# pyxploiter/HandMvNet

Measured on AMD Instinct MI355X. Metric: samples/sec (BxV frames) eval_fps.py, 8-view 256x256; 21-kpt L2 vs reference, higher is better.
Workload: dtype f32; 1 GPU; BASELINE configs[2]: B=32/GPU x V=8 x 256x256, resnet50_paper backbone, d=524, cross_attn x5, GCN decoder; global_batch=32, views=8, frame=256, parallelism=sample-shard x1

## Files before the change

handmvnet_amd/csrc/conv_stream.hip:

```cpp
#include <cstdio>
#include <cstdlib>
#include <type_traits>
#include <utility>

#include "kernels.h"

namespace hmv {

typedef float sf32x16 __attribute__((ext_vector_type(16)));
typedef float sf32x4 __attribute__((ext_vector_type(4)));
typedef _Float16 sf16x8 __attribute__((ext_vector_type(8)));

#define HMV_SGLDS16(gptr, lptr)                                                                             \
    __builtin_amdgcn_global_load_lds((const __attribute__((address_space(1))) void *)(gptr),                \
                                     (__attribute__((address_space(3))) void *)(lptr), 16, 0, 0)

template <int N>
__device__ __forceinline__ void wait_vm() {
    static_assert(N >= 0 && N < 64, "vmcnt is a 6-bit field");
    asm volatile("s_waitcnt vmcnt(%0)" ::"n"(N) : "memory");
}
template <typename F, int... I>
__device__ __forceinline__ void static_for_impl(F &&f, std::integer_sequence<int, I...>) {
    (f(std::integral_constant<int, I>{}), ...);
}
template <int N, typename F>
__device__ __forceinline__ void static_for(F &&f) {
    static_for_impl(static_cast<F &&>(f), std::make_integer_sequence<int, N>{});
}

constexpr int sched_r(int RB, int RS, int j) { return RS ? RS : (j == 0 ? RB : 0); }
constexpr int sched_ops(int NP, int PA, int RB, int RS, int OS, int slot) { return slot < NP ? PA + sched_r(RB, RS, slot) : OS; }
constexpr int sched_after_piece(int NP, int D, int PA, int RB, int RS, int OS, int j) {
    const int T0 = 8, g = T0 * NP + j - D, tq = g / NP, jq = g - tq * NP;
    int n = sched_r(RB, RS, jq);
    for (int s = tq * (NP + 1) + jq + 1; s < T0 * (NP + 1) + j; ++s) n += sched_ops(NP, PA, RB, RS, OS, s % (NP + 1));
    return n;
}
constexpr int sched_after_residual(int NP, int PA, int RB, int RS, int OS) {
    const int T0 = 8, last = RS ? NP - 1 : 0;
    int n = 0;
    for (int s = (T0 - 1) * (NP + 1) + last + 1; s < T0 * (NP + 1) + NP; ++s) n += sched_ops(NP, PA, RB, RS, OS, s % (NP + 1));
    return n;
}
static_assert(sched_after_piece(4, 3, 1, 8, 0, 8, 0) == 10 && sched_after_piece(4, 3, 1, 8, 0, 8, 1) == 18 && sched_after_piece(4, 3, 1, 8, 0, 8, 2) == 18 &&
              sched_after_piece(4, 3, 1, 8, 0, 8, 3) == 10 && sched_after_residual(4, 1, 8, 0, 8) == 23, "the step-0 schedule of four pieces, counted by hand");
static_assert(sched_after_piece(4, 3, 1, 8, 2, 8, 0) == 2 + 3 + 3 + 8 && sched_after_residual(4, 1, 8, 2, 8) == 8 + 4 * 3, "the spread K = 256 schedule");

template <int TM, int TN, int MW, int NW, int NP, int NSLOT, bool HAS_RES, bool SPREAD = false, bool DUAL = false, int N2 = 0>
__global__ __launch_bounds__(64 * MW *NW, (MW * NW) / 4) void conv_stream_f16(const ConvParams p) {
    constexpr int NWV = MW * NW, NT = 64 * NWV;
    constexpr int BM = 32 * TM * MW, BN = 32 * TN * NW;
    constexpr int D = NSLOT - 1;
    constexpr int PA = BM * 8 / NT;
    constexpr int NB2 = N2 / 32;
    constexpr int TM2 = N2 ? (BM / 32) * NB2 / NWV : 0;
    constexpr int K2Q = BN / 16;
    static_assert(N2 == 0 || (N2 % 32 == 0 && TN == 2 && TM2 >= 1 && NWV % NB2 == 0 && (BM / 32) == (NWV / NB2) * TM2),
                  "chain: a wave's 64 output channels are one pixel piece of the second reduction; whole blocks per wave");
    constexpr int RB = HAS_RES ? TM * TN * 2 : 0, OS = TM * TN * 2 + 2 * TM2;
    constexpr int RS = (SPREAD && HAS_RES) ? RB / NP : 0;
    static_assert(!SPREAD || RB % NP == 0, "spread schedule: whole residual DMAs per step");
    constexpr int ZW = TM * TN * 2 * 1024;
    constexpr int NFAKE = (D + NP - 1) / NP;
    static_assert(NT == 512 && BM % 64 == 0 && PA >= 1, "eight waves; whole DMA passes per piece");
    static_assert((NSLOT & (NSLOT - 1)) == 0 && NSLOT >= 2, "a power of two");
    extern __shared__ __attribute__((aligned(16))) char ssm[];
    _Float16 *sA = reinterpret_cast<_Float16 *>(ssm);
    char *zones = ssm + NSLOT * BM * 128;

    const int tid = threadIdx.x, lane = tid & 63;
    const int wave = __builtin_amdgcn_readfirstlane(tid >> 6);
    const int l31 = lane & 31, kh = lane >> 5;
    const int mw = wave / NW, nw = wave - mw * NW;
    const int zi = N2 ? nw * MW + mw : wave;
    static_assert(N2 == 0 || !HAS_RES || ZW == TM * 32 * 128, "chain: a landing zone is the wave's region of the tile image");

    const int nsl = p.ntiles;
    const int loc = (int)blockIdx.x >> 3, per_xcd = 32 / nsl;
    const int slice = loc % nsl, stream = ((int)blockIdx.x & 7) * per_xcd + loc / nsl, nstreams = 8 * per_xcd;
    const int ntl = p.mtiles > stream ? (p.mtiles - stream + nstreams - 1) / nstreams : 0;
    if (ntl == 0) return;
    const int n0 = slice * BN + nw * TN * 32;

    const _Float16 *zero16 = reinterpret_cast<const _Float16 *>(p.zero);
    _Float16 *trash = reinterpret_cast<_Float16 *>(const_cast<float *>(p.zero) + 64 + 4 * lane);
    const _Float16 *Ain = reinterpret_cast<const _Float16 *>(p.in);
    const _Float16 *Rin = reinterpret_cast<const _Float16 *>(p.res);
    _Float16 *Out = reinterpret_cast<_Float16 *>(p.out);

    const int wl31 = (l31 & 0x13) | ((l31 & 4) << 1) | ((l31 & 8) >> 1);
    sf16x8 wreg[TN][NP * 4];
    {
        const _Float16 *wb = reinterpret_cast<const _Float16 *>(p.wgt) + (size_t)(n0 + wl31) * p.ldw + 8 * kh;
#pragma unroll
        for (int b = 0; b < TN; ++b)
#pragma unroll
            for (int Q = 0; Q < NP * 4; ++Q) wreg[b][Q] = *reinterpret_cast<const sf16x8 *>(wb + (size_t)(32 * b) * p.ldw + 16 * Q);
    }
    const int ob2 = N2 ? wave % (N2 ? NB2 : 1) : 0, pg2 = N2 ? wave / (N2 ? NB2 : 1) : 0;
    sf16x8 w2reg[N2 ? K2Q : 1];
    if constexpr (N2 > 0) {
        const _Float16 *wb2 = reinterpret_cast<const _Float16 *>(p.nx_wgt) + (size_t)(32 * ob2 + wl31) * p.nx_ldw + 8 * kh;
#pragma unroll
        for (int Q = 0; Q < K2Q; ++Q) w2reg[Q] = *reinterpret_cast<const sf16x8 *>(wb2 + 16 * Q);
    }
    asm volatile("s_waitcnt vmcnt(0)" ::: "memory");

    const int arow = tid >> 3, kqs = (tid & 7) ^ ((tid >> 4) & 7);
    const int fsw = (l31 >> 1) & 7;

    size_t off2[DUAL ? PA : 1] = {};
    auto issue_A = [&](int G) {
        const int tt = G >= 0 ? G / NP : -1, jj = G >= 0 ? G - tt * NP : 0, slot = G & (NSLOT - 1);
        const int mt = stream + tt * nstreams;
#pragma unroll
        for (int i = 0; i < PA; ++i) {
            const int m = mt * BM + i * 64 + arow;
            const bool ok = tt >= 0 && tt < ntl && m < p.M;
            const _Float16 *src = zero16;
            if constexpr (DUAL) {
                if (jj * 64 == p.ksplit) {
                    const int hw = p.Ho * p.Wo, n = m / hw, rem = m - n * hw, ho = rem / p.Wo, wo = rem - ho * p.Wo;
                    off2[i] = ((size_t)(n * p.H2 + ho * p.stride2) * p.W2 + wo * p.stride2) * p.lda2 + 8 * kqs;
                }
                if (ok && jj * 64 >= p.ksplit) {
                    src = reinterpret_cast<const _Float16 *>(p.in2) + off2[i] + (jj * 64 - p.ksplit);
                } else if (ok) {
                    src = Ain + (size_t)m * p.lda + jj * 64 + 8 * kqs;
                }
            } else if (ok) {
                src = Ain + (size_t)m * p.lda + jj * 64 + 8 * kqs;
            }
            asm volatile("" : "+v"(src));
            HMV_SGLDS16(src, sA + ((slot * BM + i * 64 + wave * 8) * 64));
        }
    };
    auto issue_R = [&](int tt, auto first_c, auto count_c) {
        if constexpr (HAS_RES) {
            constexpr int first = decltype(first_c)::value, count = decltype(count_c)::value;
            const int mt = stream + tt * nstreams;
            char *z = zones + ((tt & 1) * NWV + zi) * ZW;
#pragma unroll
            for (int idx = first; idx < first + count; ++idx) {
                const int a = idx / (2 * TN), b = (idx / 2) % TN, j = idx & 1;
                const int m = mt * BM + (mw * TM + a) * 32 + l31;
                const bool ok = tt >= 0 && tt < ntl && m < p.M;
                const _Float16 *src = ok ? Rin + (size_t)m * p.ldr + n0 + 32 * b + 16 * j + 8 * kh : zero16;
                asm volatile("" : "+v"(src));
                HMV_SGLDS16(src, z + idx * 1024);
            }
        }
    };
    using I0 = std::integral_constant<int, 0>;
    using IRB = std::integral_constant<int, RB>;
    using IRS = std::integral_constant<int, RS>;

#pragma unroll
    for (int ft = -NFAKE; ft < 0; ++ft) {
        static_for<NP>([&](auto jc) {
            constexpr int j = decltype(jc)::value;
            issue_A(ft * NP + j + D);
            if constexpr (RS > 0) issue_R(ft + 1, std::integral_constant<int, j * RS>{}, IRS{});
            else if constexpr (j == 0) issue_R(ft + 1, I0{}, IRB{});
        });
#pragma unroll
        for (int i = 0; i < OS; ++i)
            asm volatile("global_store_dwordx4 %0, %1, off\n\ts_nop 1" ::"v"(trash), "v"(sf32x4{0.f, 0.f, 0.f, 0.f}) : "memory");
    }

    const float lo = (p.act == ACT_RELU) ? 0.f : -INFINITY;
    const __attribute__((address_space(4))) float *bp0 =
        (const __attribute__((address_space(4))) float *)(p.bias + __builtin_amdgcn_readfirstlane(n0));
    sf32x16 acc[TM][TN];

    for (int tt = 0; tt < ntl; ++tt) {
        int bz;
        asm volatile("s_mov_b32 %0, 0" : "=s"(bz));
        const __attribute__((address_space(4))) float *bp = bp0 + bz;
#pragma unroll
        for (int b = 0; b < TN; ++b)
#pragma unroll
            for (int e = 0; e < 16; ++e) {
                const int c = 32 * b + 16 * (e >> 3) + (e & 7);
                const float v0 = bp[c], v1 = bp[c + 8];
                const float v = kh ? v1 : v0;
#pragma unroll
                for (int a = 0; a < TM; ++a) acc[a][b][e] = v;
            }
        static_for<NP>([&](auto jc) {
            constexpr int j = decltype(jc)::value;
            wait_vm<sched_after_piece(NP, D, PA, RB, RS, OS, j)>();
            asm volatile("s_waitcnt lgkmcnt(0)\n\ts_barrier" ::: "memory");
            issue_A(tt * NP + j + D);
            if constexpr (RS > 0) issue_R(tt + 1, std::integral_constant<int, j * RS>{}, IRS{});
            else if constexpr (j == 0) issue_R(tt + 1, I0{}, IRB{});
            const _Float16 *pa = sA + ((((tt * NP + j) & (NSLOT - 1)) * BM + mw * TM * 32 + l31) * 64);
#pragma unroll
            for (int q = 0; q < 4; ++q) {
                sf16x8 px[TM];
#pragma unroll
                for (int a = 0; a < TM; ++a) px[a] = *reinterpret_cast<const sf16x8 *>(pa + a * 32 * 64 + (((2 * q + kh) ^ fsw) * 8));
#pragma unroll
                for (int a = 0; a < TM; ++a)
#pragma unroll
                    for (int b = 0; b < TN; ++b)
                        acc[a][b] = __builtin_amdgcn_mfma_f32_32x32x16_f16(wreg[b][4 * j + q], px[a], acc[a][b], 0, 0, 0);
            }
        });
        if constexpr (HAS_RES) wait_vm<sched_after_residual(NP, PA, RB, RS, OS)>();
        const int mt = stream + tt * nstreams;
        const char *z = zones + ((tt & 1) * NWV + zi) * ZW + lane * 16;
        if constexpr (N2 > 0) {
            char *yt = HAS_RES ? zones + (tt & 1) * NWV * ZW : zones;
            sf16x8 rr[TM][TN][2], hv[TM][TN][2];
            if constexpr (HAS_RES) {
#pragma unroll
                for (int a = 0; a < TM; ++a)
#pragma unroll
                    for (int b = 0; b < TN; ++b)
#pragma unroll
                        for (int j = 0; j < 2; ++j) rr[a][b][j] = *reinterpret_cast<const sf16x8 *>(z + ((a * TN + b) * 2 + j) * 1024);
            }
#pragma unroll
            for (int a = 0; a < TM; ++a) {
                const int m = mt * BM + (mw * TM + a) * 32 + l31;
                _Float16 *orow = Out + (size_t)m * p.ldc + n0 + 8 * kh;
#pragma unroll
                for (int b = 0; b < TN; ++b)
#pragma unroll
                    for (int j = 0; j < 2; ++j) {
                        sf16x8 r = {0, 0, 0, 0, 0, 0, 0, 0};
                        if constexpr (HAS_RES) r = rr[a][b][j];
#pragma unroll
                        for (int u = 0; u < 8; ++u) hv[a][b][j][u] = (_Float16)fmaxf(acc[a][b][8 * j + u] * p.acc_scale + (float)r[u], lo);
                        _Float16 *dst = m < p.M ? orow + 32 * b + 16 * j : trash;
                        asm volatile("global_store_dwordx4 %0, %1, off\n\ts_nop 1" ::"v"(dst), "v"(hv[a][b][j]) : "memory");
                        if constexpr (!HAS_RES) {
                            const unsigned ya = (unsigned)(size_t)(__attribute__((address_space(3))) char *)yt +
                                                (unsigned)((nw * BM + (mw * TM + a) * 32 + l31) * 128 + (((4 * b + 2 * j + kh) ^ fsw) * 16));
                            asm volatile("ds_write_b128 %0, %1" ::"v"(ya), "v"(hv[a][b][j]) : "memory");
                        }
                    }
            }
            if constexpr (HAS_RES) {
#pragma unroll
            for (int a = 0; a < TM; ++a)
#pragma unroll
                for (int b = 0; b < TN; ++b)
#pragma unroll
                    for (int j = 0; j < 2; ++j) {
                        const unsigned ya = (unsigned)(size_t)(__attribute__((address_space(3))) char *)yt +
                                            (unsigned)((nw * BM + (mw * TM + a) * 32 + l31) * 128 + (((4 * b + 2 * j + kh) ^ fsw) * 16));
                        asm volatile("ds_write_b128 %0, %1" ::"v"(ya), "v"(hv[a][b][j]) : "memory");
                    }
            }
            asm volatile("s_waitcnt lgkmcnt(0)\n\ts_barrier" ::: "memory");
            const __attribute__((address_space(4))) float *bq =
                (const __attribute__((address_space(4))) float *)(p.nx_bias + __builtin_amdgcn_readfirstlane(32 * ob2)) + bz;
            sf32x16 acc2[TM2];
#pragma unroll
            for (int e = 0; e < 16; ++e) {
                const int c = 16 * (e >> 3) + (e & 7);
                const float v0 = bq[c], v1 = bq[c + 8];
                const float v = kh ? v1 : v0;
#pragma unroll
                for (int a = 0; a < TM2; ++a) acc2[a][e] = v;
            }
            const unsigned yr = (unsigned)(size_t)(__attribute__((address_space(3))) char *)yt + (unsigned)((pg2 * TM2 * 32 + l31) * 128);
            constexpr int G = 4 / TM2, NG = K2Q / G;
            static_assert(K2Q % G == 0 && G * TM2 == 4, "four fragment reads per group");
            sf16x8 px[2][G][TM2];
#define HMV_CHAIN_READ_GROUP(g)                                                                                                     \
    _Pragma("unroll") for (int i = 0; i < G; ++i) _Pragma("unroll") for (int a = 0; a < TM2; ++a) {                                \
        const int Q = (g) * G + i;                                                                                                  \
        const unsigned ad = yr + (unsigned)(((Q >> 2) * BM + a * 32) * 128) + (unsigned)((((2 * (Q & 3) + kh) ^ fsw)) * 16);        \
        asm volatile("ds_read_b128 %0, %1" : "=v"(px[(g) & 1][i][a]) : "v"(ad) : "memory");                                         \
    }
            HMV_CHAIN_READ_GROUP(0)
#pragma unroll
            for (int g = 0; g < NG; ++g) {
                sf16x8(&pg)[G][TM2] = px[g & 1];
                if (g + 1 < NG) {
                    HMV_CHAIN_READ_GROUP(g + 1)
                    if constexpr (TM2 == 1) asm volatile("s_waitcnt lgkmcnt(4)" : "+v"(pg[0][0]), "+v"(pg[1][0]), "+v"(pg[2][0]), "+v"(pg[3][0]) :: "memory");
                    else asm volatile("s_waitcnt lgkmcnt(4)" : "+v"(pg[0][0]), "+v"(pg[0][1]), "+v"(pg[1][0]), "+v"(pg[1][1]) :: "memory");
                } else {
                    if constexpr (TM2 == 1) asm volatile("s_waitcnt lgkmcnt(0)" : "+v"(pg[0][0]), "+v"(pg[1][0]), "+v"(pg[2][0]), "+v"(pg[3][0]) :: "memory");
                    else asm volatile("s_waitcnt lgkmcnt(0)" : "+v"(pg[0][0]), "+v"(pg[0][1]), "+v"(pg[1][0]), "+v"(pg[1][1]) :: "memory");
                }
#pragma unroll
                for (int i = 0; i < G; ++i)
#pragma unroll
                    for (int a = 0; a < TM2; ++a) acc2[a] = __builtin_amdgcn_mfma_f32_32x32x16_f16(w2reg[g * G + i], pg[i][a], acc2[a], 0, 0, 0);
            }
#undef HMV_CHAIN_READ_GROUP
            const float lo2 = (p.nx_act == ACT_RELU) ? 0.f : -INFINITY;
            _Float16 *Out2 = reinterpret_cast<_Float16 *>(p.nx_out);
#pragma unroll
            for (int a = 0; a < TM2; ++a) {
                const int m = mt * BM + (pg2 * TM2 + a) * 32 + l31;
                _Float16 *orow = Out2 + (size_t)m * p.nx_ldc + 32 * ob2 + 8 * kh;
#pragma unroll
                for (int j = 0; j < 2; ++j) {
                    const sf16x8 r = {0, 0, 0, 0, 0, 0, 0, 0};
                    sf16x8 h2;
#pragma unroll
                    for (int u = 0; u < 8; ++u) h2[u] = (_Float16)fmaxf(acc2[a][8 * j + u] * p.acc_scale + (float)r[u], lo2);
                    _Float16 *dst = m < p.M ? orow + 16 * j : trash;
                    asm volatile("global_store_dwordx4 %0, %1, off\n\ts_nop 1" ::"v"(dst), "v"(h2) : "memory");
                }
            }
        } else {
#pragma unroll
        for (int a = 0; a < TM; ++a) {
            const int m = mt * BM + (mw * TM + a) * 32 + l31;
            _Float16 *orow = Out + (size_t)m * p.ldc + n0 + 8 * kh;
#pragma unroll
            for (int b = 0; b < TN; ++b)
#pragma unroll
                for (int j = 0; j < 2; ++j) {
                    sf16x8 r = {0, 0, 0, 0, 0, 0, 0, 0};
                    if constexpr (HAS_RES) r = *reinterpret_cast<const sf16x8 *>(z + ((a * TN + b) * 2 + j) * 1024);
                    sf16x8 hv;
#pragma unroll
                    for (int u = 0; u < 8; ++u) hv[u] = (_Float16)fmaxf(acc[a][b][8 * j + u] * p.acc_scale + (float)r[u], lo);
                    _Float16 *dst = m < p.M ? orow + 32 * b + 16 * j : trash;
                    asm volatile("global_store_dwordx4 %0, %1, off\n\ts_nop 1" ::"v"(dst), "v"(hv) : "memory");
                }
        }
        }
    }
    asm volatile("s_waitcnt vmcnt(0) lgkmcnt(0)" ::: "memory");
}

template <int TM, int TN, int MW, int NW, int NP, int NSLOT, bool HAS_RES, bool DUAL = false, bool HALF = false>
__global__ __launch_bounds__(64 * MW *NW, 2) void conv_stream_f32(const ConvParams p) {
    constexpr int NWV = MW * NW, NT = 64 * NWV;
    constexpr int BM = 32 * TM * MW, BN = 32 * TN * NW;
    constexpr int D = NSLOT - 1;
    constexpr int PA = BM * 8 / NT;
    constexpr int RB = HAS_RES ? TM * TN * 4 : 0, OS = TM * TN * 4, RS = 0;
    constexpr int ZW = TM * TN * 4 * 1024;
    constexpr int NFAKE = (D + NP - 1) / NP;
    constexpr int RPP = NT / 8;
    static_assert((NT == 512 || (HALF && NT == 256)) && BM % RPP == 0 && PA >= 1 && (!HALF || (HAS_RES && !DUAL)), "whole DMA passes per piece");
    static_assert((NSLOT & (NSLOT - 1)) == 0 && NSLOT >= 2, "a power of two");
    extern __shared__ __attribute__((aligned(16))) char ssm[];
    float *sA = reinterpret_cast<float *>(ssm);
    char *zones = ssm + NSLOT * BM * 128;

    const int tid = threadIdx.x, lane = tid & 63;
    const int wave = __builtin_amdgcn_readfirstlane(tid >> 6);
    const int l31 = lane & 31, kh = lane >> 5;
    const int mw = wave / NW, nw = wave - mw * NW;
    const int nsl = p.ntiles;
    const int loc = (int)blockIdx.x >> 3, per_xcd = ((int)gridDim.x >> 3) / nsl;
    const int slice = loc % nsl, stream = ((int)blockIdx.x & 7) * per_xcd + loc / nsl, nstreams = 8 * per_xcd;
    const int ntl = p.mtiles > stream ? (p.mtiles - stream + nstreams - 1) / nstreams : 0;
    if (ntl == 0) return;
    const int n0 = slice * BN + nw * TN * 32;

    const float *zero32 = p.zero;
    float *trash = const_cast<float *>(p.zero) + 64 + 4 * lane;
    const float *Ain = reinterpret_cast<const float *>(p.in);
    const float *Rin = reinterpret_cast<const float *>(p.res);
    float *Out = reinterpret_cast<float *>(p.out);

    sf32x4 wreg[TN][NP * 4], bias[TN][4];
    {
        const float *wb = reinterpret_cast<const float *>(p.wgt) + (size_t)(n0 + l31) * p.ldw + 4 * kh;
#pragma unroll
        for (int b = 0; b < TN; ++b) {
#pragma unroll
            for (int Q = 0; Q < NP * 4; ++Q) wreg[b][Q] = *reinterpret_cast<const sf32x4 *>(wb + (size_t)(32 * b) * p.ldw + 8 * Q);
#pragma unroll
            for (int g = 0; g < 4; ++g) bias[b][g] = *reinterpret_cast<const sf32x4 *>(p.bias + n0 + 32 * b + 8 * g + 4 * kh);
        }
    }
    asm volatile("s_waitcnt vmcnt(0)" ::: "memory");

    const int arow = tid >> 3, kqs = (tid & 7) ^ ((tid >> 4) & 7);
    const int fsw = (l31 >> 1) & 7;
    auto issue_A = [&](int G) {
        const int tt = G >= 0 ? G / NP : -1, jj = G >= 0 ? G - tt * NP : 0, slot = G & (NSLOT - 1);
        const int mt = stream + tt * nstreams;
#pragma unroll
        for (int i = 0; i < PA; ++i) {
            const int m = mt * BM + i * RPP + arow;
            const bool ok = tt >= 0 && tt < ntl && m < p.M;
            const float *src = zero32;
            if constexpr (DUAL) {
                if (ok && jj * 32 >= p.ksplit) {
                    const int hw = p.Ho * p.Wo, n = m / hw, rem = m - n * hw, ho = rem / p.Wo, wo = rem - ho * p.Wo;
                    src = reinterpret_cast<const float *>(p.in2) + ((size_t)(n * p.H2 + ho * p.stride2) * p.W2 + wo * p.stride2) * p.lda2 +
                          (jj * 32 - p.ksplit) + 4 * kqs;
                } else if (ok) {
                    src = Ain + (size_t)m * p.lda + jj * 32 + 4 * kqs;
                }
            } else if (ok) {
                src = Ain + (size_t)m * p.lda + jj * 32 + 4 * kqs;
            }
            asm volatile("" : "+v"(src));
            HMV_SGLDS16(src, sA + ((slot * BM + i * RPP + wave * 8) * 32));
        }
    };
    auto issue_R = [&](int tt) {
        if constexpr (HAS_RES) {
            const int mt = stream + tt * nstreams;
            char *z = zones + ((HALF ? 0 : (tt & 1)) * NWV + wave) * ZW;
#pragma unroll
            for (int idx = 0; idx < RB; ++idx) {
                const int a = idx / (4 * TN), b = (idx / 4) % TN, g = idx & 3;
                const int m = mt * BM + (mw * TM + a) * 32 + l31;
                const bool ok = tt >= 0 && tt < ntl && m < p.M;
                const float *src = ok ? Rin + (size_t)m * p.ldr + n0 + 32 * b + 8 * g + 4 * kh : zero32;
                asm volatile("" : "+v"(src));
                HMV_SGLDS16(src, z + idx * 1024);
            }
        }
    };
#pragma unroll
    for (int ft = -NFAKE; ft < 0; ++ft) {
        static_for<NP>([&](auto jc) {
            constexpr int j = decltype(jc)::value;
            issue_A(ft * NP + j + D);
            if constexpr (j == 0) issue_R(HALF ? ft : ft + 1);
        });
#pragma unroll
        for (int i = 0; i < OS; ++i)
            asm volatile("global_store_dwordx4 %0, %1, off\n\ts_nop 1" ::"v"(trash), "v"(sf32x4{0.f, 0.f, 0.f, 0.f}) : "memory");
    }

    const float lo = (p.act == ACT_RELU) ? 0.f : -INFINITY;
    sf32x16 acc[TM][TN];
    for (int tt = 0; tt < ntl; ++tt) {
#pragma unroll
        for (int a = 0; a < TM; ++a)
#pragma unroll
            for (int b = 0; b < TN; ++b)
#pragma unroll
                for (int e = 0; e < 16; ++e) acc[a][b][e] = 0.f;
        static_for<NP>([&](auto jc) {
            constexpr int j = decltype(jc)::value;
            wait_vm<sched_after_piece(NP, D, PA, RB, RS, OS, j)>();
            asm volatile("s_waitcnt lgkmcnt(0)\n\ts_barrier" ::: "memory");
            issue_A(tt * NP + j + D);
            if constexpr (j == 0) issue_R(HALF ? tt : tt + 1);
            const float *pa = sA + ((((tt * NP + j) & (NSLOT - 1)) * BM + mw * TM * 32 + l31) * 32);
#pragma unroll
            for (int q = 0; q < 4; ++q) {
                sf32x4 px[TM];
#pragma unroll
                for (int a = 0; a < TM; ++a) px[a] = *reinterpret_cast<const sf32x4 *>(pa + a * 32 * 32 + (((2 * q + kh) ^ fsw) * 4));
#pragma unroll
                for (int e = 0; e < 4; ++e)
#pragma unroll
                    for (int a = 0; a < TM; ++a)
#pragma unroll
                        for (int b = 0; b < TN; ++b)
                            acc[a][b] = __builtin_amdgcn_mfma_f32_32x32x2f32(wreg[b][4 * j + q][e], px[a][e], acc[a][b], 0, 0, 0);
            }
        });
        if constexpr (HAS_RES) wait_vm<HALF ? (NP - 1) * PA : sched_after_residual(NP, PA, RB, RS, OS)>();
        const int mt = stream + tt * nstreams;
        const char *z = zones + ((HALF ? 0 : (tt & 1)) * NWV + wave) * ZW + lane * 16;
#pragma unroll
        for (int a = 0; a < TM; ++a) {
            const int m = mt * BM + (mw * TM + a) * 32 + l31;
            float *orow = Out + (size_t)m * p.ldc + n0 + 4 * kh;
#pragma unroll
            for (int b = 0; b < TN; ++b)
#pragma unroll
                for (int g = 0; g < 4; ++g) {
                    sf32x4 r = {0.f, 0.f, 0.f, 0.f};
                    if constexpr (HAS_RES) r = *reinterpret_cast<const sf32x4 *>(z + ((a * TN + b) * 4 + g) * 1024);
                    sf32x4 t;
#pragma unroll
                    for (int u = 0; u < 4; ++u) t[u] = fmaxf((acc[a][b][4 * g + u] + bias[b][g][u]) + r[u], lo);
                    float *dst = m < p.M ? orow + 32 * b + 8 * g : trash;
                    asm volatile("global_store_dwordx4 %0, %1, off\n\ts_nop 1" ::"v"(dst), "v"(t) : "memory");
                }
        }
    }
    asm volatile("s_waitcnt vmcnt(0) lgkmcnt(0)" ::: "memory");
}

template <int TM, int TN, int MW, int NW, int NP, int NSLOT, bool HAS_RES, bool SPREAD = false, bool DUAL = false, int N2 = 0>
static hipError_t launch_stream_one(ConvParams p, hipStream_t s) {
    constexpr int BM = 32 * TM * MW, BN = 32 * TN * NW, NWV = MW * NW;
    constexpr size_t lds = (size_t)NSLOT * BM * 128 + (HAS_RES ? (size_t)2 * NWV * TM * TN * 2 * 1024 : (N2 ? (size_t)BM * BN * 2 : 0));
    static_assert(lds <= 160 * 1024, "LDS budget");
    auto kern = conv_stream_f16<TM, TN, MW, NW, NP, NSLOT, HAS_RES, SPREAD, DUAL, N2>;
    if (N2 && (p.Cout != BN || p.nx_cout != N2 || !p.nx_wgt || !p.nx_bias || !p.nx_out)) return hipErrorInvalidValue;
    static DeviceOnce once;
    if (const hipError_t e = once.run([&](int) { return set_max_lds(lds, kern); }); e != hipSuccess) return e;
    p.mtiles = (p.M + BM - 1) / BM;
    p.ntiles = p.Cout / BN;
    hipLaunchKernelGGL(kern, dim3(256), dim3(64 * NWV), lds, s, p);
    return hipGetLastError();
}

static int stream_bn(const ConvParams &p, int *bm = nullptr) {
    int bn = 0, m = 0;
    if (p.in2) {
        if (!p.res && p.Kpad == 128 && p.ksplit == 64 && p.Cout == 256) { bn = 256; m = 128; }
        else if (!p.res && p.Kpad == 384 && p.ksplit == 128 && p.Cout == 512) { bn = 256; m = 64; }
    } else if (p.res) {
        if (p.Kpad == 256 || p.Kpad == 128) { bn = 512; m = 64; }
        else if (p.Kpad == 64) { bn = 256; m = 128; }
    } else {
        if (p.Kpad == 256 && p.Cout == 64) { bn = 64; m = 256; }
        else if (p.Kpad == 512 && p.Cout == 128) { bn = 128; m = 128; }
        else if (p.Kpad == 256 && p.Cout == 128) { bn = 128; m = 128; }
        else if (p.Kpad == 64 && p.Cout == 64) { bn = 64; m = 256; }
    }
    if (bm) *bm = m;
    return bn;
}

static int stream32_shape(const ConvParams &p) {
    if (p.in_f16 || p.out_f16) return 0;
    if (p.in2) return (!p.res && p.Kpad == 128 && p.ksplit == 64 && p.Cout == 256 && p.lda == p.ksplit && p.lda2 % 4 == 0) ? 3 : 0;
    if (p.res) return (!p.res_f16 && (p.Kpad == 64 || p.Kpad == 128 || p.Kpad == 256) && p.Cout % 256 == 0 && 32 % (p.Cout / 256) == 0) ? 1 : 0;
    return (p.Kpad == 256 && p.Cout == 64) ? 2 : ((p.Kpad == 64 && p.Cout == 64) ? 4 : 0);
}
static bool stream32_rule(const ConvParams &p) {
    static const bool no256 = HMV_DEV_ENV("HMV_NO_STREAM32_K256") != nullptr;
    return p.res ? (p.Kpad <= 128 || (!no256 && p.Cout % 128 == 0 && 64 % (p.Cout / 128) == 0)) : true;
}

bool conv_stream_supported(const ConvParams &p, const ConvRoute &route) {
    static const int min_env = HMV_DEV_INT("HMV_STREAM_MIN_TILES", 4);
    if (route.stream == ROUTE_NEVER) return false;
    const bool force = route.stream == ROUTE_FORCE;
    const int min_tiles = force ? 0 : min_env;
    if (stream32_shape(p)) {
        static const bool off32 = HMV_DEV_ENV("HMV_NO_STREAM32") != nullptr;
        if (off32 && !force) return false;
        if (p.R != 1 || p.S != 1 || p.stride != 1 || p.pad_h || p.pad_w || p.up || p.ksl > 1 || p.phases > 1) return false;
        if (p.cwrap || p.x3_plane || p.res_split || p.out_split || p.acc_shift || p.rd_cout || p.scatter || p.rg_out || p.fill) return false;
        if (p.act != ACT_NONE && p.act != ACT_RELU) return false;
        if ((!p.in2 && p.Cin != p.Kpad) || p.K != p.Kpad) return false;
        if ((p.lda ? p.lda : p.Cin) % 4 || (p.ldw ? p.ldw : p.Kpad) % 4 || p.ldc % 4 || (p.res && p.ldr % 4)) return false;
        if (force) return true;
        const int bm32 = (p.res || p.in2) ? 64 : 128, streams32 = p.res ? 256 / (p.Cout / 256) : 256;
        return stream32_rule(p) && (long long)(p.M + bm32 - 1) / bm32 >= (long long)min_tiles * streams32;
    }
    int bm = 0;
    const int bn = stream_bn(p, &bm);
    if (!bn || !p.in_f16 || !p.out_f16 || (p.res && !p.res_f16)) return false;
    if (p.R != 1 || p.S != 1 || p.stride != 1 || p.pad_h || p.pad_w || p.up || p.ksl > 1 || p.phases > 1) return false;
    if (p.in2 && ((p.lda2 & 7) || (p.ksplit & 63) || p.lda != p.ksplit)) return false;
    if (p.cwrap || p.x3_plane || p.res_split || p.out_split || p.acc_shift || p.rd_cout || p.scatter || p.rg_out || p.fill) return false;
    if (p.act != ACT_NONE && p.act != ACT_RELU) return false;
    if ((!p.in2 && p.Cin != p.Kpad) || p.K != p.Kpad || p.Cout % bn != 0 || 32 % (p.Cout / bn) != 0) return false;
    if ((p.lda ? p.lda : p.Cin) % 8 || (p.ldw ? p.ldw : p.Kpad) % 8 || p.ldc % 8 || (p.res && p.ldr % 8)) return false;
    const int streams = 256 / (p.Cout / bn);
    return (long long)(p.M + bm - 1) / bm >= (long long)min_tiles * streams;
}

bool conv_stream_chain_ok(const ConvParams &q, int nx_cout, const ConvRoute &route) {
    static const bool off = HMV_DEV_ENV("HMV_NO_CHAIN") != nullptr;
    if (off || (nx_cout != 64 && nx_cout != 128)) return false;
    ConvParams p = q;
    p.nx_wgt = nullptr;
    if (!p.lda) p.lda = p.Cin;
    if (!p.ldw) p.ldw = p.Kpad;
    if (!p.in_f16 || !p.out_f16 || p.acc_shift || p.Cout != 256 || (p.ldc & 7)) return false;
    if (!(p.in2 ? (!p.res && p.Kpad == 128 && p.ksplit == 64 && nx_cout == 64) : (p.res && p.Kpad == 64))) return false;
    return conv_stream_supported(p, route);
}

template <int TM, int TN, int MW, int NW, int NP, int NSLOT, bool HAS_RES, bool DUAL = false, bool HALF = false>
static hipError_t launch_stream32(ConvParams p, hipStream_t s) {
    constexpr int BM = 32 * TM * MW, BN = 32 * TN * NW;
    constexpr size_t lds = (size_t)NSLOT * BM * 128 + (HAS_RES ? (size_t)(HALF ? 1 : 2) * MW * NW * TM * TN * 4 * 1024 : 0);
    static_assert(lds * (HALF ? 2 : 1) <= 160 * 1024, "LDS budget");
    auto kern = conv_stream_f32<TM, TN, MW, NW, NP, NSLOT, HAS_RES, DUAL, HALF>;
    static DeviceOnce once;
    if (const hipError_t e = once.run([&](int) { return set_max_lds(lds, kern); }); e != hipSuccess) return e;
    p.mtiles = (p.M + BM - 1) / BM;
    p.ntiles = p.Cout / BN;
    hipLaunchKernelGGL(kern, dim3(HALF ? 512 : 256), dim3(64 * MW * NW), lds, s, p);
    return hipGetLastError();
}

hipError_t launch_conv_stream(const ConvParams &p, hipStream_t s, const char **name) {
    if (const int k32 = stream32_shape(p)) {
        if (k32 == 2) { if (name) *name = "conv_stream_f32<128x64,k256>"; return launch_stream32<1, 1, 4, 2, 8, 8, false>(p, s); }
        if (k32 == 4) { if (name) *name = "conv_stream_f32<128x64,k64>"; return launch_stream32<1, 1, 4, 2, 2, 8, false>(p, s); }
        if (k32 == 3) { if (name) *name = "conv_stream_f32<64x256,k128,dual>"; return launch_stream32<2, 1, 1, 8, 4, 8, false, true>(p, s); }
        if (p.Kpad == 256 && p.Cout % 128 == 0 && 64 % (p.Cout / 128) == 0) {
            if (name) *name = "conv_stream_f32<64x128,k256,res>";
            return launch_stream32<2, 1, 1, 4, 8, 4, true, false, true>(p, s);
        }
        if (p.Kpad == 256) { if (name) *name = "conv_stream_f32<64x256,k256,res>"; return launch_stream32<2, 1, 1, 8, 8, 4, true>(p, s); }
        if (p.Kpad == 128) { if (name) *name = "conv_stream_f32<64x256,k128,res>"; return launch_stream32<2, 1, 1, 8, 4, 4, true>(p, s); }
        if (name) *name = "conv_stream_f32<64x256,k64,res>";
        return launch_stream32<2, 1, 1, 8, 2, 4, true>(p, s);
    }
    if (p.nx_wgt) {
        if (p.nx_ldw < p.Cout || (p.nx_ldw & 7) || (p.nx_ldc & 7) || (p.nx_act != ACT_NONE && p.nx_act != ACT_RELU) || p.acc_shift) return hipErrorInvalidValue;
        if (p.in2 && p.Kpad == 128 && p.nx_cout == 64) {
            if (name) *name = "conv_stream_f16<128x256,k128,dual,+1x1:64>";
            return launch_stream_one<2, 2, 2, 4, 2, 4, false, false, true, 64>(p, s);
        }
        if (p.res && p.Kpad == 64 && p.nx_cout == 64) {
            if (name) *name = "conv_stream_f16<128x256,k64,res,+1x1:64>";
            return launch_stream_one<2, 2, 2, 4, 1, 2, true, false, false, 64>(p, s);
        }
        if (p.res && p.Kpad == 64 && p.nx_cout == 128) {
            if (name) *name = "conv_stream_f16<128x256,k64,res,+1x1:128>";
            return launch_stream_one<2, 2, 2, 4, 1, 2, true, false, false, 128>(p, s);
        }
        return hipErrorInvalidValue;
    }
    if (p.in2) {
        if (p.Kpad == 128) {
            if (name) *name = "conv_stream_f16<128x256,k128,dual>";
            return launch_stream_one<2, 2, 2, 4, 2, 8, false, false, true>(p, s);
        }
        if (name) *name = "conv_stream_f16<64x256,k384,dual>";
        return launch_stream_one<2, 1, 1, 8, 6, 8, false, false, true>(p, s);
    }
    if (!p.res) {
        if (p.Kpad == 256 && p.Cout == 64) {
            if (name) *name = "conv_stream_f16<256x64,k256>";
            return launch_stream_one<1, 2, 8, 1, 4, 4, false>(p, s);
        }
        if (p.Kpad == 64 && p.Cout == 64) {
            if (name) *name = "conv_stream_f16<256x64,k64>";
            return launch_stream_one<1, 2, 8, 1, 1, 4, false>(p, s);
        }
        if (p.Kpad == 512) {
            if (name) *name = "conv_stream_f16<128x128,k512>";
            return launch_stream_one<2, 1, 2, 4, 8, 8, false>(p, s);
        }
        if (name) *name = "conv_stream_f16<128x128,k256>";
        return launch_stream_one<1, 2, 4, 2, 4, 8, false>(p, s);
    }
    if (p.Kpad == 256) {
        if (name) *name = "conv_stream_f16<64x512,k256,res>";
        return launch_stream_one<2, 2, 1, 8, 4, 4, true, true>(p, s);
    }
    if (p.Kpad == 128) {
        if (name) *name = "conv_stream_f16<64x512,k128,res>";
        return launch_stream_one<2, 2, 1, 8, 2, 4, true>(p, s);
    }
    if (p.Kpad == 64) {
        if (name) *name = "conv_stream_f16<128x256,k64,res>";
        return launch_stream_one<2, 2, 2, 4, 1, 2, true>(p, s);
    }
    return hipErrorInvalidValue;
}

}
```

Measured before the change: 5960 frames/s.

## Group pieces per barrier and software-pipeline LDS fragment reads in f32 stream conv

Adds a PB (pieces per barrier) mode to the f32 streaming conv, so several K-pieces share one wait and barrier. Within a step, LDS fragments are double-buffered with explicit ds_read_b128, overlapping reads with the MFMAs, and a LATE option defers the DMA issue until after the first MFMA group. The mode is enabled by default for the k128 dual (PB=4, LATE) and k128 residual (PB=2) shapes. Dev-only phase timers and env-selected variants are also added. Fewer barriers and overlapped LDS latency are meant to cut stalls, at the cost of a shallower prefetch distance and more registers.

```diff
diff --git a/handmvnet_amd/csrc/conv_stream.hip b/handmvnet_amd/csrc/conv_stream.hip
--- a/handmvnet_amd/csrc/conv_stream.hip
+++ b/handmvnet_amd/csrc/conv_stream.hip
@@ -46,6 +46,10 @@
 static_assert(sched_after_piece(4, 3, 1, 8, 0, 8, 0) == 10 && sched_after_piece(4, 3, 1, 8, 0, 8, 1) == 18 && sched_after_piece(4, 3, 1, 8, 0, 8, 2) == 18 &&
               sched_after_piece(4, 3, 1, 8, 0, 8, 3) == 10 && sched_after_residual(4, 1, 8, 0, 8) == 23, "the step-0 schedule of four pieces, counted by hand");
 static_assert(sched_after_piece(4, 3, 1, 8, 2, 8, 0) == 2 + 3 + 3 + 8 && sched_after_residual(4, 1, 8, 2, 8) == 8 + 4 * 3, "the spread K = 256 schedule");
+static_assert(sched_after_piece(4, 1, 4, 8, 0, 8, 0) == 8 && sched_after_piece(4, 1, 4, 8, 0, 8, 1) == 8 && sched_after_piece(4, 1, 4, 8, 0, 8, 2) == 0 &&
+              sched_after_piece(4, 1, 4, 8, 0, 8, 3) == 0, "two pieces per barrier, one step ahead, counted by hand");
+static_assert(sched_after_piece(2, 1, 2, 8, 0, 8, 0) == 8 && sched_after_piece(2, 1, 2, 8, 0, 8, 1) == 8 && sched_after_residual(2, 2, 8, 0, 8) == 2 + 8 + 2 + 8 + 2,
+              "K = 128 with a residual, two pieces per barrier, counted by hand");
 
 template <int TM, int TN, int MW, int NW, int NP, int NSLOT, bool HAS_RES, bool SPREAD = false, bool DUAL = false, int N2 = 0>
 __global__ __launch_bounds__(64 * MW *NW, (MW * NW) / 4) void conv_stream_f16(const ConvParams p) {
@@ -334,15 +338,18 @@
     asm volatile("s_waitcnt vmcnt(0) lgkmcnt(0)" ::: "memory");
 }
 
-template <int TM, int TN, int MW, int NW, int NP, int NSLOT, bool HAS_RES, bool DUAL = false, bool HALF = false>
+template <int TM, int TN, int MW, int NW, int NP, int NSLOT, bool HAS_RES, bool DUAL = false, bool HALF = false, int PB = 0, bool LATE = false>
 __global__ __launch_bounds__(64 * MW *NW, 2) void conv_stream_f32(const ConvParams p) {
     constexpr int NWV = MW * NW, NT = 64 * NWV;
     constexpr int BM = 32 * TM * MW, BN = 32 * TN * NW;
-    constexpr int D = NSLOT - 1;
+    constexpr int PBS = PB ? PB : 1;
+    constexpr int NS = NP / PBS, DS = NSLOT / PBS - 1;
+    constexpr int D = NSLOT - PBS;
+    static_assert(NP % PBS == 0 && NSLOT % PBS == 0 && DS >= 1 && (!LATE || PB > 0), "whole steps per tile and per ring");
     constexpr int PA = BM * 8 / NT;
     constexpr int RB = HAS_RES ? TM * TN * 4 : 0, OS = TM * TN * 4, RS = 0;
     constexpr int ZW = TM * TN * 4 * 1024;
-    constexpr int NFAKE = (D + NP - 1) / NP;
+    constexpr int NFAKE = (DS + NS - 1) / NS;
     constexpr int RPP = NT / 8;
     static_assert((NT == 512 || (HALF && NT == 256)) && BM % RPP == 0 && PA >= 1 && (!HALF || (HAS_RES && !DUAL)), "whole DMA passes per piece");
     static_assert((NSLOT & (NSLOT - 1)) == 0 && NSLOT >= 2, "a power of two");
@@ -425,7 +432,7 @@
         static_for<NP>([&](auto jc) {
             constexpr int j = decltype(jc)::value;
             issue_A(ft * NP + j + D);
-            if constexpr (j == 0) issue_R(HALF ? ft : ft + 1);
+            if constexpr (j == PBS - 1) issue_R(HALF ? ft : ft + 1);
         });
 #pragma unroll
         for (int i = 0; i < OS; ++i)
@@ -433,7 +440,24 @@
     }
 
     const float lo = (p.act == ACT_RELU) ? 0.f : -INFINITY;
+    using I0 = std::integral_constant<int, 0>;
+#ifdef HMV_DEV_KNOBS
+    unsigned long long ph[5] = {0, 0, 0, 0, 0}, ph_ts = 0, ph_t0 = 0;
+    const bool ph_on = p.dbg != nullptr;
+    if (ph_on) ph_ts = ph_t0 = __builtin_amdgcn_s_memtime();
+#define HMV_PHASE(i)                                                       \
+    if (ph_on) {                                                           \
+        __builtin_amdgcn_sched_barrier(0);                                 \
+        const unsigned long long ph_now = __builtin_amdgcn_s_memtime();    \
+        ph[i] += ph_now - ph_ts;                                           \
+        ph_ts = ph_now;                                                    \
+        __builtin_amdgcn_sched_barrier(0);                                 \
+    }
+#else
+#define HMV_PHASE(i)
+#endif
     sf32x16 acc[TM][TN];
+    sf32x4 fx[2][TM];
     for (int tt = 0; tt < ntl; ++tt) {
 #pragma unroll
         for (int a = 0; a < TM; ++a)
@@ -441,28 +465,89 @@
             for (int b = 0; b < TN; ++b)
 #pragma unroll
                 for (int e = 0; e < 16; ++e) acc[a][b][e] = 0.f;
-        static_for<NP>([&](auto jc) {
-            constexpr int j = decltype(jc)::value;
-            wait_vm<sched_after_piece(NP, D, PA, RB, RS, OS, j)>();
-            asm volatile("s_waitcnt lgkmcnt(0)\n\ts_barrier" ::: "memory");
-            issue_A(tt * NP + j + D);
-            if constexpr (j == 0) issue_R(HALF ? tt : tt + 1);
-            const float *pa = sA + ((((tt * NP + j) & (NSLOT - 1)) * BM + mw * TM * 32 + l31) * 32);
-#pragma unroll
-            for (int q = 0; q < 4; ++q) {
-                sf32x4 px[TM];
-#pragma unroll
-                for (int a = 0; a < TM; ++a) px[a] = *reinterpret_cast<const sf32x4 *>(pa + a * 32 * 32 + (((2 * q + kh) ^ fsw) * 4));
-#pragma unroll
-                for (int e = 0; e < 4; ++e)
-#pragma unroll
-                    for (int a = 0; a < TM; ++a)
-#pragma unroll
-                        for (int b = 0; b < TN; ++b)
-                            acc[a][b] = __builtin_amdgcn_mfma_f32_32x32x2f32(wreg[b][4 * j + q][e], px[a][e], acc[a][b], 0, 0, 0);
-            }
-        });
-        if constexpr (HAS_RES) wait_vm<HALF ? (NP - 1) * PA : sched_after_residual(NP, PA, RB, RS, OS)>();
+        if constexpr (PB == 0) {
+            static_for<NP>([&](auto jc) {
+                constexpr int j = decltype(jc)::value;
+                HMV_PHASE(j == 0 ? 4 : 3)
+                wait_vm<sched_after_piece(NP, D, PA, RB, RS, OS, j)>();
+                HMV_PHASE(0)
+                asm volatile("s_waitcnt lgkmcnt(0)\n\ts_barrier" ::: "memory");
+                HMV_PHASE(1)
+                issue_A(tt * NP + j + D);
+                if constexpr (j == 0) issue_R(HALF ? tt : tt + 1);
+                const float *pa = sA + ((((tt * NP + j) & (NSLOT - 1)) * BM + mw * TM * 32 + l31) * 32);
+                HMV_PHASE(2)
+#pragma unroll
+                for (int q = 0; q < 4; ++q) {
+                    sf32x4 px[TM];
+#pragma unroll
+                    for (int a = 0; a < TM; ++a) px[a] = *reinterpret_cast<const sf32x4 *>(pa + a * 32 * 32 + (((2 * q + kh) ^ fsw) * 4));
+#pragma unroll
+                    for (int e = 0; e < 4; ++e)
+#pragma unroll
+                        for (int a = 0; a < TM; ++a)
+#pragma unroll
+                            for (int b = 0; b < TN; ++b)
+                                acc[a][b] = __builtin_amdgcn_mfma_f32_32x32x2f32(wreg[b][4 * j + q][e], px[a][e], acc[a][b], 0, 0, 0);
+                }
+            });
+        } else {
+            static_for<NS>([&](auto sc) {
+                constexpr int s = decltype(sc)::value;
+                HMV_PHASE(s == 0 ? 4 : 3)
+                wait_vm<sched_after_piece(NS, DS, PA * PBS, RB, RS, OS, s)>();
+                HMV_PHASE(0)
+                asm volatile("s_waitcnt lgkmcnt(0)\n\ts_barrier" ::: "memory");
+                HMV_PHASE(1)
+                unsigned pa[PBS];
+#pragma unroll
+                for (int i = 0; i < PBS; ++i)
+                    pa[i] = (unsigned)(size_t)(__attribute__((address_space(3))) char *)ssm + (unsigned)((((tt * NP + s * PBS + i) & (NSLOT - 1)) * BM + mw * TM * 32 + l31) * 128);
+                static_assert(TM == 1 || TM == 2, "fragment sets of one or two blocks");
+                auto read_group = [&](sf32x4(&st)[TM], auto qc) {
+                    constexpr int qg = decltype(qc)::value;
+                    const unsigned ad = pa[qg >> 2] + (unsigned)(((2 * (qg & 3) + kh) ^ fsw) * 16);
+                    asm volatile("ds_read_b128 %0, %1" : "=v"(st[0]) : "v"(ad) : "memory");
+                    if constexpr (TM == 2) asm volatile("ds_read_b128 %0, %1 offset:%2" : "=v"(st[TM - 1]) : "v"(ad), "n"(32 * 128) : "memory");
+                };
+                auto wait_group = [](sf32x4(&st)[TM]) {
+                    if constexpr (TM == 1) asm volatile("s_waitcnt lgkmcnt(0)" : "+v"(st[0]) :: "memory");
+                    else asm volatile("s_waitcnt lgkmcnt(0)" : "+v"(st[0]), "+v"(st[TM - 1]) :: "memory");
+                };
+                read_group(fx[0], I0{});
+                __builtin_amdgcn_sched_barrier(0);
+                auto issue_step = [&]() {
+#pragma unroll
+                    for (int i = 0; i < PBS; ++i) issue_A(tt * NP + s * PBS + i + D);
+                    if constexpr (s == 0) issue_R(HALF ? tt : tt + 1);
+                };
+                if constexpr (!LATE) issue_step();
+                wait_group(fx[0]);
+                __builtin_amdgcn_sched_barrier(0);
+                HMV_PHASE(2)
+                static_for<4 * PBS>([&](auto qc) {
+                    constexpr int qq = decltype(qc)::value, cur = qq & 1;
+                    if constexpr (qq + 1 < 4 * PBS) read_group(fx[cur ^ 1], std::integral_constant<int, qq + 1>{});
+                    __builtin_amdgcn_sched_barrier(0);
+#pragma unroll
+                    for (int e = 0; e < 4; ++e)
+#pragma unroll
+                        for (int a = 0; a < TM; ++a)
+#pragma unroll
+                            for (int b = 0; b < TN; ++b)
+                                acc[a][b] = __builtin_amdgcn_mfma_f32_32x32x2f32(wreg[b][4 * s * PBS + qq][e], fx[cur][a][e], acc[a][b], 0, 0, 0);
+                    __builtin_amdgcn_sched_barrier(0);
+                    if constexpr (LATE && qq == 0) {
+                        issue_step();
+                        __builtin_amdgcn_sched_barrier(0);
+                    }
+                    if constexpr (qq + 1 < 4 * PBS) wait_group(fx[cur ^ 1]);
+                    __builtin_amdgcn_sched_barrier(0);
+                });
+            });
+        }
+        HMV_PHASE(3)
+        if constexpr (HAS_RES) wait_vm<HALF ? (NS - 1) * PA * PBS : sched_after_residual(NS, PA * PBS, RB, RS, OS)>();
         const int mt = stream + tt * nstreams;
         const char *z = zones + ((HALF ? 0 : (tt & 1)) * NWV + wave) * ZW + lane * 16;
 #pragma unroll
@@ -483,6 +568,19 @@
                 }
         }
     }
+#ifdef HMV_DEV_KNOBS
+    if (ph_on) {
+        HMV_PHASE(4)
+        if (blockIdx.x == 0 && lane == 0) {
+            unsigned long long *d = p.dbg + 8 * wave;
+            for (int i = 0; i < 5; ++i) d[i] = ph[i];
+            d[5] = (unsigned long long)ntl;
+            d[6] = ph_ts - ph_t0;
+            d[7] = 0;
+        }
+    }
+#endif
+#undef HMV_PHASE
     asm volatile("s_waitcnt vmcnt(0) lgkmcnt(0)" ::: "memory");
 }
 
@@ -572,12 +670,12 @@
     return conv_stream_supported(p, route);
 }
 
-template <int TM, int TN, int MW, int NW, int NP, int NSLOT, bool HAS_RES, bool DUAL = false, bool HALF = false>
+template <int TM, int TN, int MW, int NW, int NP, int NSLOT, bool HAS_RES, bool DUAL = false, bool HALF = false, int PB = 0, bool LATE = false>
 static hipError_t launch_stream32(ConvParams p, hipStream_t s) {
     constexpr int BM = 32 * TM * MW, BN = 32 * TN * NW;
     constexpr size_t lds = (size_t)NSLOT * BM * 128 + (HAS_RES ? (size_t)(HALF ? 1 : 2) * MW * NW * TM * TN * 4 * 1024 : 0);
     static_assert(lds * (HALF ? 2 : 1) <= 160 * 1024, "LDS budget");
-    auto kern = conv_stream_f32<TM, TN, MW, NW, NP, NSLOT, HAS_RES, DUAL, HALF>;
+    auto kern = conv_stream_f32<TM, TN, MW, NW, NP, NSLOT, HAS_RES, DUAL, HALF, PB, LATE>;
     static DeviceOnce once;
     if (const hipError_t e = once.run([&](int) { return set_max_lds(lds, kern); }); e != hipSuccess) return e;
     p.mtiles = (p.M + BM - 1) / BM;
@@ -588,15 +686,43 @@
 
 hipError_t launch_conv_stream(const ConvParams &p, hipStream_t s, const char **name) {
     if (const int k32 = stream32_shape(p)) {
-        if (k32 == 2) { if (name) *name = "conv_stream_f32<128x64,k256>"; return launch_stream32<1, 1, 4, 2, 8, 8, false>(p, s); }
+#ifdef HMV_DEV_KNOBS
+        static const int step = HMV_DEV_INT("HMV_STREAM32_STEP", -1);
+#define HMV_S32_FORM(n, ...) if (step == n) return launch_stream32<__VA_ARGS__>(p, s);
+#else
+#define HMV_S32_FORM(n, ...)
+#endif
+        if (k32 == 2) {
+            if (name) *name = "conv_stream_f32<128x64,k256>";
+            HMV_S32_FORM(0, 1, 1, 4, 2, 8, 8, false) HMV_S32_FORM(1, 1, 1, 4, 2, 8, 8, false, false, false, 1)
+            HMV_S32_FORM(2, 1, 1, 4, 2, 8, 8, false, false, false, 2) HMV_S32_FORM(3, 1, 1, 4, 2, 8, 8, false, false, false, 4)
+            HMV_S32_FORM(5, 1, 1, 4, 2, 8, 8, false, false, false, 2, true) HMV_S32_FORM(6, 1, 1, 4, 2, 8, 8, false, false, false, 4, true)
+            return launch_stream32<1, 1, 4, 2, 8, 8, false>(p, s);
+        }
         if (k32 == 4) { if (name) *name = "conv_stream_f32<128x64,k64>"; return launch_stream32<1, 1, 4, 2, 2, 8, false>(p, s); }
-        if (k32 == 3) { if (name) *name = "conv_stream_f32<64x256,k128,dual>"; return launch_stream32<2, 1, 1, 8, 4, 8, false, true>(p, s); }
+        if (k32 == 3) {
+            if (name) *name = "conv_stream_f32<64x256,k128,dual>";
+            HMV_S32_FORM(0, 2, 1, 1, 8, 4, 8, false, true) HMV_S32_FORM(1, 2, 1, 1, 8, 4, 8, false, true, false, 1)
+            HMV_S32_FORM(2, 2, 1, 1, 8, 4, 8, false, true, false, 2) HMV_S32_FORM(3, 2, 1, 1, 8, 4, 8, false, true, false, 4)
+            HMV_S32_FORM(5, 2, 1, 1, 8, 4, 8, false, true, false, 4, true) HMV_S32_FORM(6, 2, 1, 1, 8, 4, 8, false, true, false, 2, true)
+            return launch_stream32<2, 1, 1, 8, 4, 8, false, true, false, 4, true>(p, s);
+        }
         if (p.Kpad == 256 && p.Cout % 128 == 0 && 64 % (p.Cout / 128) == 0) {
             if (name) *name = "conv_stream_f32<64x128,k256,res>";
+            HMV_S32_FORM(0, 2, 1, 1, 4, 8, 4, true, false, true) HMV_S32_FORM(1, 2, 1, 1, 4, 8, 4, true, false, true, 1)
+            HMV_S32_FORM(2, 2, 1, 1, 4, 8, 4, true, false, true, 2)
+            HMV_S32_FORM(5, 2, 1, 1, 4, 8, 4, true, false, true, 1, true) HMV_S32_FORM(6, 2, 1, 1, 4, 8, 4, true, false, true, 2, true)
             return launch_stream32<2, 1, 1, 4, 8, 4, true, false, true>(p, s);
         }
         if (p.Kpad == 256) { if (name) *name = "conv_stream_f32<64x256,k256,res>"; return launch_stream32<2, 1, 1, 8, 8, 4, true>(p, s); }
-        if (p.Kpad == 128) { if (name) *name = "conv_stream_f32<64x256,k128,res>"; return launch_stream32<2, 1, 1, 8, 4, 4, true>(p, s); }
+        if (p.Kpad == 128) {
+            if (name) *name = "conv_stream_f32<64x256,k128,res>";
+            HMV_S32_FORM(0, 2, 1, 1, 8, 4, 4, true) HMV_S32_FORM(1, 2, 1, 1, 8, 4, 4, true, false, false, 1)
+            HMV_S32_FORM(2, 2, 1, 1, 8, 4, 4, true, false, false, 2) HMV_S32_FORM(3, 2, 1, 1, 8, 4, 4, true, false, false, 2)
+            HMV_S32_FORM(5, 2, 1, 1, 8, 4, 4, true, false, false, 2, true) HMV_S32_FORM(6, 2, 1, 1, 8, 4, 4, true, false, false, 1, true)
+            return launch_stream32<2, 1, 1, 8, 4, 4, true, false, false, 2>(p, s);
+        }
+#undef HMV_S32_FORM
         if (name) *name = "conv_stream_f32<64x256,k64,res>";
         return launch_stream32<2, 1, 1, 8, 2, 4, true>(p, s);
     }
```

Measured after the change: 5973 frames/s (median of 6 runs). No clear change (+0.2%).
